# Yzmblog/SurfD

Measured on AMD Instinct MI355X. Metric: shapes/sec end-to-end (1000-step uncond, 512^3 UDF) at 1/2/4/8 GPU, higher is better.
Workload: dtype f32 (every matrix product of decoder and denoiser as three split-fp16 products on the fp16 MFMA pipe with fp32 accumulation — fp32-class error, same golden tolerances as the exact-fp32 kernels; samplers, attention, embedding MLP and grid bookkeeping in exact fp32)

## Files before the change

surfd_amd/csrc/unet.hip:

```cpp
#include "common.h"
#include "unet_api.h"
#include "unet_plan.h"
#include <string.h>
#include <algorithm>
#include <stdlib.h>

namespace surfd {

struct SegArgs {
    const float *x;
    long bstride;
    int C, Cp;
    int Lin;
    int taps, stride, ups;
    int gn, act;
    int bmod;
    const float *gamma, *beta;
    int kg_off;
    int cc;
    const float *add;
    long add_step_stride;
};

struct ConvArgs {
// ... 422 lines not shown
            const int ct = ct0 + i * ct_step;
            if (ct >= nct) continue;
            const int m = ct * 32 + (lane & 31);
            const bool mok = m < M;
            const int b = b0 + (m >> A.log2Lout), l = m & (A.Lout - 1);
            float add[16];
#pragma unroll
            for (int r = 0; r < 16; ++r) {
                if constexpr (NTW == 1) {
                    add[r] = pre_add[r];
                } else {
                    const int co = tile * 32 + frag_row(r, lane);
                    const bool ok = mok && co < A.Cout;
                    float t = 0.f;
                    if (ok) {
                        if (A.bias) t = A.bias[co];
                        if (embp) t += embp[b * A.emb_bstride + co];
                        if (A.res) t += A.res[b * A.res_bstride + (long)co * A.Lout + l];
                    }
                    add[r] = t;
                }
            }
#pragma unroll
            for (int r = 0; r < 16; ++r) {
                const int co = tile * 32 + frag_row(r, lane);
                if (mok && co < A.Cout) A.out[b * A.out_bstride + (long)co * A.Lout + l] = acc[i][r] + add[r];
            }
        }
    }
    if (dbg_on) { asm volatile("s_waitcnt vmcnt(0)" ::: "memory"); DBG_STAMP(9); }
#undef DBG_STAMP
}

__global__ __launch_bounds__(256) void attn_kernel(const float *qkv, long qkv_bstride, float *out, long out_bstride,
                                                   int heads, int d, int T, float scale) {
    extern __shared__ __attribute__((aligned(16))) float lds[];
    const int qt_n = (T + 31) >> 5;
    const int bh = blockIdx.x / qt_n, qt = blockIdx.x - bh * qt_n;
    const int b = bh / heads, h = bh - b * heads;
    const int tid = threadIdx.x, lane = tid & 63, col = lane & 31, half = lane >> 5;
    const int wave = __builtin_amdgcn_readfirstlane(tid >> 6);
    const int Tp = T + 1;
    float *q = lds, *k = q + d * Tp, *v = k + d * Tp;
    float *xch = v + d * Tp;
    if (T & 3) {
        const float *src = qkv + b * qkv_bstride + (long)h * 3 * d * T;
        for (int e = tid; e < 3 * d * T; e += 256) {
            const int c = e / T, t = e - c * T;
            lds[c * Tp + t] = c < 2 * d ? src[e] * scale : src[e];
        }
    } else {
        const f32x4 *src4 = reinterpret_cast<const f32x4 *>(qkv + b * qkv_bstride + (long)h * 3 * d * T);
        const int vpr = T >> 2, n4 = 3 * d * vpr;
        for (int e = tid; e < n4; e += 256) {
            const int c = e / vpr, t4 = e - c * vpr;
            f32x4 x = src4[e];
            if (c < 2 * d) { x[0] *= scale; x[1] *= scale; x[2] *= scale; x[3] *= scale; }
            float *dstp = lds + c * Tp + 4 * t4;
            dstp[0] = x[0]; dstp[1] = x[1]; dstp[2] = x[2]; dstp[3] = x[3];
        }
    }
    __syncthreads();
    const int t_glob = qt * 32 + col;
    const bool t_ok = t_glob < T;
    f32x16 sc[2];
#pragma unroll
    for (int kt = 0; kt < 2; ++kt)
#pragma unroll
        for (int r = 0; r < 16; ++r) sc[kt][r] = 0.f;
    const int cper = ((d / 2 + 3) / 4) * 2;
    const int c_beg = wave * cper, c_end = min(d, c_beg + cper);
    for (int c = c_beg; c < c_end; c += 2) {
        const float qv = t_ok ? q[(c + half) * Tp + t_glob] : 0.f;
#pragma unroll
        for (int kt = 0; kt < 2; ++kt)
            if (kt < qt_n) {
                const int s_ = kt * 32 + col;
                const float kv = s_ < T ? k[(c + half) * Tp + s_] : 0.f;
                sc[kt] = __builtin_amdgcn_mfma_f32_32x32x2f32(kv, qv, sc[kt], 0, 0, 0);
            }
    }
#pragma unroll
    for (int kt = 0; kt < 2; ++kt)
        if (kt < qt_n)
#pragma unroll
            for (int r = 0; r < 16; ++r) xch[((wave * qt_n + kt) * 16 + r) * 64 + lane] = sc[kt][r];
    __syncthreads();
#pragma unroll
    for (int kt = 0; kt < 2; ++kt)
        if (kt < qt_n)
#pragma unroll
            for (int r = 0; r < 16; ++r) {
                float t = 0.f;
#pragma unroll
                for (int w = 0; w < 4; ++w) t += xch[((w * qt_n + kt) * 16 + r) * 64 + lane];
                sc[kt][r] = t;
            }
    float mx = -INFINITY;
#pragma unroll
    for (int kt = 0; kt < 2; ++kt)
        if (kt < qt_n)
#pragma unroll
            for (int r = 0; r < 16; ++r) {
                const int s_ = kt * 32 + frag_row(r, lane);
                if (s_ >= T) sc[kt][r] = -INFINITY;
                mx = fmaxf(mx, sc[kt][r]);
            }
    mx = fmaxf(mx, __shfl_xor(mx, 32));
    float sum = 0.f;
#pragma unroll
    for (int kt = 0; kt < 2; ++kt)
        if (kt < qt_n)
#pragma unroll
            for (int r = 0; r < 16; ++r) { const float ex = expf(sc[kt][r] - mx); sc[kt][r] = ex; sum += ex; }
    sum += __shfl_xor(sum, 32);
#pragma unroll
    for (int kt = 0; kt < 2; ++kt)
#pragma unroll
        for (int r = 0; r < 16; ++r) sc[kt][r] = sc[kt][r] / sum;
    float *dst = out + b * out_bstride + (long)h * d * T;
    for (int c0 = wave * 32; c0 < d; c0 += 128) {
        f32x16 acc;
#pragma unroll
        for (int r = 0; r < 16; ++r) acc[r] = 0.f;
        const int c = c0 + col;
#pragma unroll
        for (int kt = 0; kt < 2; ++kt)
            if (kt < qt_n)
#pragma unroll
                for (int r = 0; r < 16; ++r) {
                    const int s_ = kt * 32 + frag_row(r, lane);
                    const float vv = (c < d && s_ < T) ? v[c * Tp + s_] : 0.f;
                    acc = __builtin_amdgcn_mfma_f32_32x32x2f32(vv, sc[kt][r], acc, 0, 0, 0);
                }
        if (t_ok)
#pragma unroll
            for (int r = 0; r < 16; ++r) {
                const int cr = c0 + frag_row(r, lane);
                if (cr < d) dst[(long)cr * T + t_glob] = acc[r];
            }
    }
}

__global__ void temb_kernel(const int64_t *t, int rows, int dim, float *out) {
    const int half = dim / 2;
    for (int e = blockIdx.x * blockDim.x + threadIdx.x; e < rows * half; e += gridDim.x * blockDim.x) {
        const int r = e / half, kk = e % half;
        const float freq = expf(__fdiv_rn(__fmul_rn(-9.210340371976184f, (float)kk), (float)half));
        const float a = __fmul_rn((float)t[r], freq);
        out[(long)r * dim + kk] = cosf(a);
        out[(long)r * dim + half + kk] = sinf(a);
    }
}

__global__ void add_label_kernel(float *emb, int rows, int dim, const float *table, const int64_t *cls, int B) {
    for (long e = blockIdx.x * (long)blockDim.x + threadIdx.x; e < (long)rows * dim; e += (long)gridDim.x * blockDim.x) {
        const int r = (int)(e / dim), c = (int)(e % dim);
        emb[e] += table[cls[r % B] * dim + c];
    }
}

__global__ void vec_add_kernel(float *dst, const float *a, const float *b, int n) {
    for (int e = blockIdx.x * blockDim.x + threadIdx.x; e < n; e += gridDim.x * blockDim.x) dst[e] = a[e] + (b ? b[e] : 0.f);
}

}

using namespace surfd;

namespace {

void add_param(surfd_unet *u, const std::string &k, std::vector<int64_t> shape) {
    u->pindex[k] = (int)u->params.size();
    u->params.push_back({k, std::move(shape)});
// ... 710 lines not shown
}

int unet_prepare_embeddings(surfd_unet *u, const int64_t *t_rows_host, int rows, const float *ctx, const int64_t *cls,
                            int B, hipStream_t st, bool shared) {
    if (rows > u->t_cap) {
        if (u->t_dev) HIP_TRY(hipFree(u->t_dev));
        u->t_dev = nullptr;
        HIP_TRY(hipMalloc((void **)&u->t_dev, (size_t)rows * sizeof(int64_t)));
        u->t_cap = rows;
    }
    HIP_TRY(hipMemcpyAsync(u->t_dev, t_rows_host, (size_t)rows * sizeof(int64_t), hipMemcpyHostToDevice, st));
    HIP_TRY(hipStreamSynchronize(st));
    return unet_prepare_embeddings_dev(u, u->t_dev, rows, ctx, cls, B, st, shared);
}

LoopState *unet_loop_state(surfd_unet *u) { return &u->loop; }
int unet_device(surfd_unet *u) { return u->device; }
long unet_workspace_generation(surfd_unet *u) { return u->ws_gen; }

static int run_op(surfd_unet *u, const Op &op, const float *x, float *out, int B, int L, const float *emb, hipStream_t st,
                  const int *step_ptr, const LoopFuse *lf = nullptr, bool *lf_done = nullptr) {
    if (op.kind == 0) {
        const float *in[2] = {x, x}; const long bs[2] = {(long)u->cfg.in_channels * L, (long)u->cfg.in_channels * L};
        const int bm[2] = {0, 0};
        return launch_conv(u, op.conv, B, L, in, bs, bm, out, (long)u->cfg.out_channels * L, emb, u->emb_total, st, step_ptr, lf, lf_done);
    }
    const AttnPlan &a = op.attn;
    const int T = L / a.ds, heads = u->cfg.num_heads, d = a.C / heads;
    const float *qkv = u->buf_ptr[a.qkv.buf];
    float *o = u->buf_ptr[a.out.buf];
    const long qbs = (long)u->bufs[a.qkv.buf].C * T, obs = (long)u->bufs[a.out.buf].C * T;
    const float scale = 1.f / sqrtf(sqrtf((float)d));
    if (T > 64) SURFD_FAIL(SURFD_ERR_UNSUPPORTED, "attention: sequence length %d (at most 64 positions per attention block)", T);
    const int qtn = (T + 31) / 32;
    const size_t lds_bytes = ((size_t)3 * d * (T + 1) + (size_t)4 * qtn * 16 * 64) * sizeof(float);
    hipLaunchKernelGGL(attn_kernel, dim3(B * heads * qtn), dim3(256), lds_bytes, st, qkv, qbs, o, obs, heads, d, T, scale);
    LAUNCH_CHECK();
    return SURFD_OK;
}

int unet_forward_prepared(surfd_unet *u, const float *x, int row0, float *out, int B, int L, hipStream_t st,
                          const int *step_ptr, const LoopFuse *lf, bool *lf_done) {
    if (!u->finalized) SURFD_FAIL(SURFD_ERR_STATE, "unet: parameters not finalized");
    if (row0 < 0 || row0 + (u->emb_shared ? 1 : B) > u->emb_rows) SURFD_FAIL(SURFD_ERR_STATE, "unet: embedding rows [%d,%d) not prepared", row0, row0 + B);
    if (u->emb_ingraph && (row0 != 0 || B != u->emb_B)) SURFD_FAIL(SURFD_ERR_STATE, "unet: in-loop embedding rows were prepared for %d samples", u->emb_B);
    int max_ds = 1;
    for (auto &b : u->bufs) max_ds = std::max(max_ds, b.ds);
    if (L % max_ds || L < max_ds || L > 64 || (L & (L - 1))) SURFD_FAIL(SURFD_ERR_UNSUPPORTED, "unet: latent length %d must be a power of two in [%d, 64]", L, max_ds);
    int rc = ensure_workspace(u, B, L);
    if (rc) return rc;
    const float *emb = u->emb_table + (size_t)row0 * u->emb_total;
    if (u->emb_ingraph) {
        const float *in[2] = {u->emb_ctx, nullptr}; const long bs[2] = {u->ted, 0}; const int bm[2] = {0, 0};
        if ((rc = launch_conv(u, u->lin3, B, 1, in, bs, bm, u->emb_table, u->emb_total, nullptr, 0, st, step_ptr, nullptr, nullptr, u->emb, u->ted))) return rc;
    }
    const ConvPlan *first_conv = nullptr;
    for (auto &op : u->ops) if (op.kind == 0) { first_conv = &op.conv; break; }
    for (size_t i = 0; i < u->ops.size(); ++i) {
        u->pf_next = first_conv;
        for (size_t j = i + 1; j < u->ops.size(); ++j) if (u->ops[j].kind == 0) { u->pf_next = &u->ops[j].conv; break; }
        rc = run_op(u, u->ops[i], x, out, B, L, emb, st, step_ptr, lf, lf_done);
        u->pf_next = nullptr;
        if (rc) return rc;
    }
    return SURFD_OK;
}
// ... 96 lines not shown
```

surfd_amd/csrc/decoder.hip:

```cpp
#include "common.h"
#include "points.h"
#include <string.h>
#include <stdlib.h>
#include <type_traits>
#include <utility>

namespace surfd {

constexpr int H = 512;
constexpr int NB = 5;
constexpr int NCBN = 2 * NB + 1;
constexpr int TP = 64;
constexpr int XS = H + 4;
constexpr int ES = 68;
constexpr int KG_H = H / 8;
constexpr int KG_E = 8;

constexpr size_t SZ_FCP = (size_t)16 * KG_E * 256;
constexpr size_t SZ_HH = (size_t)16 * KG_H * 256;
constexpr size_t SZ_FCPT = (size_t)2 * KG_H * 256;
constexpr size_t OFF_FCP = 0;
__host__ __device__ constexpr size_t off_fc(int k, int which) { return SZ_FCP + (size_t)(2 * k + which) * SZ_HH; }
__host__ __device__ constexpr size_t off_fcT(int k, int which) { return SZ_FCP + (size_t)(2 * NB + 2 * k + which) * SZ_HH; }
constexpr size_t OFF_FCPT = SZ_FCP + (size_t)4 * NB * SZ_HH;
constexpr size_t WPACK_FLOATS = OFF_FCPT + SZ_FCPT;
constexpr int VOFF_BFCP = 0;
__host__ __device__ constexpr int voff_bfc(int k, int which) { return H * (1 + 2 * k + which); }
constexpr int VOFF_WOUT = H * (1 + 2 * NB);
constexpr int VOFF_BOUT = H * (2 + 2 * NB);
__host__ __device__ constexpr int voff_cb(int k) { return VOFF_BOUT + 4 + H * k; }
constexpr int VEC_FLOATS = VOFF_BOUT + 4 + H * (NB + 1);

typedef _Float16 f16x8 __attribute__((ext_vector_type(8)));
typedef _Float16 f16x2 __attribute__((ext_vector_type(2)));
// ... 1002 lines not shown
    const __attribute__((address_space(1))) char *wb = (const __attribute__((address_space(1))) char *)(((unsigned long long)whi << 32) | wlo);
#pragma unroll
    for (int nt = 0; nt < 2; ++nt)
#pragma unroll
        for (int q = 0; q < 2; ++q)
#if defined(SURFD_DEC_W_NT) && SURFD_DEC_W_NT
            dst[nt][q] = __builtin_nontemporal_load(reinterpret_cast<const gf16x8 *>(wb + (size_t)(nt * KS * 2048) + (lofs + (unsigned)((ks * 2 + q) * 1024))));
#else
            dst[nt][q] = *reinterpret_cast<const gf16x8 *>(wb + (size_t)(nt * KS * 2048) + (lofs + (unsigned)((ks * 2 + q) * 1024)));
#endif
}

__device__ __forceinline__ void mfma_step8(const f16x8 (&a)[2][2], const f16x8 (&b)[2][2], f32x16 (&acc)[2][2]) {
    constexpr int TA[3] = {1, 0, 0};
    constexpr int TB[3] = {0, 1, 0};
#pragma unroll
    for (int t = 0; t < 3; ++t)
#pragma unroll
        for (int nt = 0; nt < 2; ++nt)
#pragma unroll
            for (int mt = 0; mt < 2; ++mt)
                acc[mt][nt] = __builtin_amdgcn_mfma_f32_32x32x16_f16(a[mt][TA[t]], b[nt][TB[t]], acc[mt][nt], 0, 0, 0);
}

template <int KS>
__device__ __forceinline__ void gemm8_request(WStages8 &ws, const _Float16 *Whf, int lane) {
    __builtin_amdgcn_sched_barrier(0);
    unsigned lofs = (unsigned)lane * 16u;
    asm volatile("" : "+v"(lofs));
    load_wstage8<KS>(ws.b[0], Whf, lofs, 0);
    __builtin_amdgcn_sched_barrier(0);
}

template <int KS>
__device__ __forceinline__ void gemm8(const float *A, const _Float16 *Whf, WStages8 &ws, f32x16 (&acc)[2][2], int lane) {
    constexpr int D = 4;
    static_assert(KS % D == 0, "k-step count must be a multiple of the pipeline depth");
    const float *a0 = A + (lane & 31) * XS + 4 * (lane >> 5);
    const float *a1 = a0 + 32 * XS;
    unsigned lofs = (unsigned)lane * 16u;
    asm volatile("" : "+v"(lofs));
    f16x8 x[2][2][2];
    auto group = [&](int ks0, auto last) {
        int goff = ks0 * 8;
        asm volatile("" : "+v"(goff));
#pragma unroll
        for (int j = 0; j < D; ++j) {
            if (!decltype(last)::value || j == 0) load_wstage8<KS>(ws.b[(j + D - 1) % D], Whf, lofs, ks0 + j + D - 1);
            const int jn = (decltype(last)::value && j == D - 1) ? j : j + 1;
            x[(j + 1) & 1][0][0] = *reinterpret_cast<const f16x8 *>(a0 + goff + jn * 8); x[(j + 1) & 1][0][1] = *reinterpret_cast<const f16x8 *>(a0 + goff + 256 + jn * 8);
            x[(j + 1) & 1][1][0] = *reinterpret_cast<const f16x8 *>(a1 + goff + jn * 8); x[(j + 1) & 1][1][1] = *reinterpret_cast<const f16x8 *>(a1 + goff + 256 + jn * 8);
            mfma_step8(x[j & 1], ws.b[j], acc);
#pragma unroll
            for (int i = 0; i < 4; ++i) { __builtin_amdgcn_sched_group_barrier(0x008, 1, 0); __builtin_amdgcn_sched_group_barrier(0x020, 1, 0); }
#pragma unroll
            for (int i = 0; i < 4; ++i) { __builtin_amdgcn_sched_group_barrier(0x008, 1, 0); __builtin_amdgcn_sched_group_barrier(0x100, 1, 0); }
            __builtin_amdgcn_sched_group_barrier(0x008, 4, 0);
            __builtin_amdgcn_sched_barrier(0);
        }
    };
    x[0][0][0] = *reinterpret_cast<const f16x8 *>(a0); x[0][0][1] = *reinterpret_cast<const f16x8 *>(a0 + 256);
    x[0][1][0] = *reinterpret_cast<const f16x8 *>(a1); x[0][1][1] = *reinterpret_cast<const f16x8 *>(a1 + 256);
    if constexpr (KS > D) {
#pragma unroll
        for (int d = 1; d < D - 1; ++d) load_wstage8<KS>(ws.b[d], Whf, lofs, d);
#pragma unroll 1
        for (int ks0 = 0; ks0 < KS - D; ks0 += D) group(ks0, std::false_type{});
        group(KS - D, std::true_type{});
    } else {
#pragma unroll
        for (int d = 1; d < D; ++d) load_wstage8<KS>(ws.b[d], Whf, lofs, d);
        int goff = 0;
        asm volatile("" : "+v"(goff));
#pragma unroll
        for (int j = 0; j < D; ++j) {
            const int jn = j == D - 1 ? j : j + 1;
            x[(j + 1) & 1][0][0] = *reinterpret_cast<const f16x8 *>(a0 + goff + jn * 8); x[(j + 1) & 1][0][1] = *reinterpret_cast<const f16x8 *>(a0 + goff + 256 + jn * 8);
            x[(j + 1) & 1][1][0] = *reinterpret_cast<const f16x8 *>(a1 + goff + jn * 8); x[(j + 1) & 1][1][1] = *reinterpret_cast<const f16x8 *>(a1 + goff + 256 + jn * 8);
            mfma_step8(x[j & 1], ws.b[j], acc);
            __builtin_amdgcn_sched_barrier(0);
        }
    }
}

__global__ __launch_bounds__(512, 1) void decoder_fwd8_kernel(DecParams P, PtBatch B) {
    extern __shared__ __attribute__((aligned(16))) float lds[];
    float *X = lds;
    float *PT = lds + TP * XS;
    float *LOG = PT + TP * 4;
    const int tid = threadIdx.x, lane = tid & 63, wave = tid >> 6;
    const int col = lane & 31;
    const int wave_u = __builtin_amdgcn_readfirstlane(wave);
    float *const xb0 = X + (4 * (lane >> 5)) * XS + 64 * wave + col;
    float *const xb1 = xb0 + 32 * XS;
#define XAT8(mt, nt, r) ((mt) ? xb1 : xb0)[(((r) & 3) + 8 * ((r) >> 2)) * XS + 32 * (nt)]
    typedef unsigned __attribute__((address_space(3))) lds_u32;
    lds_u32 *xw0 = (lds_u32 *)(reinterpret_cast<unsigned *>(X) + (4 * (lane >> 5)) * XS + 32 * wave + col);
    lds_u32 *xw1 = xw0 + 32 * XS;
#define XW8(mt, r, pl) ((mt) ? xw1 : xw0)[(((r) & 3) + 8 * ((r) >> 2)) * XS + 256 * (pl)]
#ifndef SURFD_DEC_XCD_STAGGER
#define SURFD_DEC_XCD_STAGGER 0
#endif
#if SURFD_DEC_XCD_STAGGER > 0
    for (int k_ = 0; k_ < (int)(blockIdx.x & 7) * SURFD_DEC_XCD_STAGGER; ++k_) __builtin_amdgcn_s_sleep(127);
#endif
#ifndef SURFD_DEC_CLOCK
#define SURFD_DEC_CLOCK 1
#endif
#if SURFD_DEC_CLOCK
    unsigned long long *const clk = reinterpret_cast<unsigned long long *>(P.sat + 2);
    unsigned long long *const clk0 = reinterpret_cast<unsigned long long *>(LOG + TP);
    if (blockIdx.x == 0 && tid == 0) {
        clk0[0] = (unsigned long long)__builtin_readcyclecounter();
        clk0[1] = (unsigned long long)__builtin_amdgcn_s_memrealtime();
    }
#endif
    int sat_flag = 0;
    auto store8 = [&](const f32x16 (&v)[2][2], const float (&sa)[2], const float (&sb)[2]) {
        float umax = 0.f;
#pragma unroll
        for (int mt = 0; mt < 2; ++mt)
#pragma unroll
            for (int r = 0; r < 16; ++r) {
                const float t0 = __builtin_fmaf(sa[0], v[mt][0][r], sb[0]);
                const float t1 = __builtin_fmaf(sa[1], v[mt][1][r], sb[1]);
                umax = __builtin_fmaxf(__builtin_fmaxf(umax, t0), t1);
                const float u0 = __builtin_amdgcn_fmed3f(t0, 0.f, 65504.f);
                const float u1 = __builtin_amdgcn_fmed3f(t1, 0.f, 65504.f);
                const f32x2 u = {u0, u1};
                const unsigned h = __builtin_bit_cast(unsigned, __builtin_convertvector(u, f16x2));
                XW8(mt, r, 0) = h;
                XW8(mt, r, 1) = split_low_pair(h, u0, u1);
            }
        sat_flag |= __any(umax > 65504.f);
    };
    auto zero8 = [](f32x16 (&a)[2][2]) {
#pragma unroll
        for (int mt = 0; mt < 2; ++mt)
#pragma unroll
            for (int nt = 0; nt < 2; ++nt)
#pragma unroll
                for (int r = 0; r < 16; ++r) a[mt][nt][r] = 0.f;
    };
    WStages8 ws;
    for (int bi = 0; bi < B.n; ++bi) {
    const PtIO &io = B.io[bi];
    const long npts = pt_count(io);
    const long ntiles = (npts + TP - 1) / TP;
    const float *tab_sample = P.tab + (size_t)B.sample[bi] * NCBN * 2 * H;
    const long tstep = io.shard_n > 1 ? io.shard_n : 1;
    for (long tile = blockIdx.x * tstep + (io.shard_n > 1 ? io.shard_i : 0); tile < ntiles; tile += gridDim.x * tstep) {
        const long e0 = tile * TP;
        const float *vecs_ = P.vecs, *tab_ = tab_sample;
        const _Float16 *whf = P.whf;
        unsigned cb = 64 * wave + col;
        asm volatile("" : "+s"(vecs_), "+s"(tab_), "+s"(whf), "+v"(cb), "+v"(xw0), "+v"(xw1));
        const gfloat *vecs = (const gfloat *)vecs_, *tab = (const gfloat *)tab_;
        const size_t woff_e = (size_t)(2 * wave_u) * KS_E * 2 * 512, woff = (size_t)(2 * wave_u) * KS_H * 2 * 512;
        __syncthreads();
        {
        int tid_fe = threadIdx.x;
        asm volatile("" : "+v"(tid_fe));
        const int tid = tid_fe;
        if (tid < TP) {
            const long e = e0 + tid;
            float x = 0.f, y = 0.f, z = 0.f;
            int vox = -1;
            if (e < npts) {
                if (io.mode == PT_XYZ) { x = io.xyz[e * 3 + 0]; y = io.xyz[e * 3 + 1]; z = io.xyz[e * 3 + 2]; vox = 0; }
                else if (io.mode == PT_EMB) vox = 0;
                else { vox = pt_voxel(io, e); voxel_xyz(io, vox, x, y, z); }
            }
            PT[tid * 4 + 0] = x; PT[tid * 4 + 1] = y; PT[tid * 4 + 2] = z;
            PT[tid * 4 + 3] = __int_as_float(vox);
        }
        __syncthreads();
        encode_tile_f16x2<8>(io, e0, npts, PT, X, tid, sat_flag);
        }
        gemm8_request<KS_E>(ws, whf + woff_e, lane);
        __syncthreads();
        f32x16 net[2][2], tmp[2][2];
        zero8(net);
        const float winv = vecs[VOFF_SC + 1];
        float nsa[2], nsb[2];
#pragma unroll
        for (int nt = 0; nt < 2; ++nt) {
            const unsigned c = cb + 32 * nt;
            const float a = tab[c];
            nsa[nt] = a * winv;
            nsb[nt] = __builtin_fmaf(a, vecs[voff_cb(0) + c], tab[H + c]);
        }
        gemm8<KS_E>(X, whf + woff_e, ws, net, lane);
        __syncthreads();
#pragma unroll 1
        for (int k = 0; k < NB; ++k) {
            const _Float16 *W0 = whf + (HF_FCP + (size_t)(2 * k) * HF_HH) + woff, *W1 = W0 + HF_HH;
            {
                float sa[2] = {nsa[0], nsa[1]}, sb[2] = {nsb[0], nsb[1]};
                store8(net, sa, sb);
            }
            gemm8_request<KS_H>(ws, W0, lane);
            __syncthreads();
            zero8(tmp);
            float sa1[2], sbb[2];
#pragma unroll
            for (int nt = 0; nt < 2; ++nt) {
                const unsigned c = cb + 32 * nt;
                const float a = tab[(2 * k + 1) * 2 * H + c];
                sa1[nt] = a * winv;
                sbb[nt] = __builtin_fmaf(a, vecs[H * (1 + 2 * k) + c], tab[(2 * k + 1) * 2 * H + H + c]);
            }
            gemm8<KS_H>(X, W0, ws, tmp, lane);
            __syncthreads();
            store8(tmp, sa1, sbb);
            gemm8_request<KS_H>(ws, W1, lane);
            __syncthreads();
#pragma unroll
            for (int nt = 0; nt < 2; ++nt) {
                const unsigned c = cb + 32 * nt;
                const float a = tab[(2 * k + 2) * 2 * H + c];
                nsa[nt] = a * winv;
                nsb[nt] = __builtin_fmaf(a, vecs[voff_cb(0) + H * (k + 1) + c], tab[(2 * k + 2) * 2 * H + H + c]);
            }
            gemm8<KS_H>(X, W1, ws, net, lane);
            __syncthreads();
        }
        {
#pragma unroll
            for (int nt = 0; nt < 2; ++nt) {
                const float wo = vecs[VOFF_WOUT + cb + 32 * nt];
#pragma unroll
                for (int mt = 0; mt < 2; ++mt)
#pragma unroll
                    for (int r = 0; r < 16; ++r) {
                        const float u = nsa[nt] * net[mt][nt][r] + nsb[nt];
                        XAT8(mt, nt, r) = fmaxf(u, 0.f) * wo;
                    }
            }
        }
        __syncthreads();
        {
            const float bo = vecs[VOFF_BOUT];
            for (int pp = 0; pp < TP / 8; ++pp) {
                const int p = wave * (TP / 8) + pp;
                float sacc = 0.f;
#pragma unroll
                for (int i = 0; i < H / 64; ++i) sacc += X[p * XS + lane + 64 * i];
#pragma unroll
                for (int off = 32; off > 0; off >>= 1) sacc += __shfl_xor(sacc, off);
                if (lane == 0) LOG[p] = sacc + bo;
            }
        }
        __syncthreads();
        if (tid < TP) {
            const long e = e0 + tid;
            const bool valid = e < npts;
            float udf = 0.f;
            int vox = 0;
            if (valid) {
                const float o = LOG[tid];
                const float y = 1.f / (1.f + expf(-o));
                udf = (1.f - y) * 0.1f;
                if (io.out_logit) io.out_logit[e] = o;
                if (io.out_udf) io.out_udf[e] = udf;
                if (io.grid_udf) {
                    vox = __float_as_int(PT[tid * 4 + 3]);
                    io.grid_udf[vox] = udf;
                }
            }
            if (io.grid_udf && io.grad_list) {
                const int slot = wave_append_slot(io.grad_count, valid && udf < io.grad_thr);
                if (slot >= 0) io.grad_list[slot] = vox;
            }
        }
    }
    }
    if (sat_flag && lane == 0) atomicAdd(P.sat, 1u);
#if SURFD_DEC_CLOCK
    if (blockIdx.x == 0 && tid == 0) {
        const unsigned long long c1 = (unsigned long long)__builtin_readcyclecounter(), r1 = (unsigned long long)__builtin_amdgcn_s_memrealtime();
        atomicAdd(clk + 2, c1 - clk0[0]);
        atomicAdd(clk + 3, r1 - clk0[1]);
    }
#endif
}
#undef XAT8
#undef XW8

#undef XW
constexpr size_t DEC_LDS_BYTES = (size_t)(TP * XS + TP * 4 + TP + TP * ES + TP * 4 + 4) * sizeof(float);

__global__ void absmax_kernel(const float *src, size_t n, unsigned *out) {
    unsigned m = 0u;
    for (size_t i = blockIdx.x * (size_t)blockDim.x + threadIdx.x; i < n; i += (size_t)gridDim.x * blockDim.x)
        m = max(m, __float_as_uint(src[i]) & 0x7fffffffu);
#pragma unroll
    for (int off = 32; off > 0; off >>= 1) m = max(m, (unsigned)__shfl_xor((int)m, off));
    if ((threadIdx.x & 63) == 0 && m) atomicMax(out, m);
}

__global__ void weight_scale_kernel(const unsigned *maxbits, float *sc) {
    const unsigned b = *maxbits;
    int e = (int)(b >> 23) - 127;
    if (b == 0u || e > 100 || e < -100) e = 8;
    sc[0] = __uint_as_float((unsigned)(127 + 8 - e) << 23);
    sc[1] = __uint_as_float((unsigned)(127 - 8 + e) << 23);
}
// ... 454 lines not shown
```

Before: 4.924.

## Specialize attention kernel on sequence length and batch LDS loads

Moves the attention body into a templated core specialized by sequence length, so that only the needed score fragment rows are reduced, exponentiated and multiplied for short sequences. The global-to-LDS staging now issues four loads per thread before any stores and uses shift and mask indexing in place of division. The QK loop preloads eight channel pairs from LDS ahead of the MFMAs, and waves that own no output channels exit after the exchange barrier. A power-of-two check on T is added to protect the shift indexing. Attention is a small share of the UNet, so the end-to-end effect is likely limited.

```diff
diff --git a/surfd_amd/csrc/unet.hip b/surfd_amd/csrc/unet.hip
--- a/surfd_amd/csrc/unet.hip
+++ b/surfd_amd/csrc/unet.hip
@@ -478,114 +478,155 @@
 #undef DBG_STAMP
 }
 
+template <int NR, int KT, class Sink>
+__device__ __forceinline__ void attn_core_tile(float *lds, const float *src, int d, int T, int qt, float scale, Sink &&sink) {
+    constexpr int qt_n = KT;
+    const int tid = threadIdx.x, lane = tid & 63, col = lane & 31, half = lane >> 5;
+    const int wave = __builtin_amdgcn_readfirstlane(tid >> 6);
+    const int Tp = T + 1;
+    float *q = lds, *k = q + d * Tp, *v = k + d * Tp;
+    float *xch = v + d * Tp;
+    if (T & 3) {
+        const int lt = __builtin_ctz(T), n = 3 * d * T;
+        for (int e0 = tid; e0 < n; e0 += 1024) {
+            float x[4];
+#pragma unroll
+            for (int j = 0; j < 4; ++j) x[j] = src[min(e0 + 256 * j, n - 1)];
+#pragma unroll
+            for (int j = 0; j < 4; ++j) asm volatile("" : "+v"(x[j]));
+#pragma unroll
+            for (int j = 0; j < 4; ++j) {
+                const int e = e0 + 256 * j;
+                const int c = e >> lt, t = e & (T - 1);
+                if (e < n) lds[c * Tp + t] = c < 2 * d ? x[j] * scale : x[j];
+            }
+        }
+    } else {
+        const f32x4 *src4 = reinterpret_cast<const f32x4 *>(src);
+        const int vpr = T >> 2, lv = __builtin_ctz(vpr), n4 = 3 * d * vpr;
+        for (int e0 = tid; e0 < n4; e0 += 1024) {
+            f32x4 xs[4];
+#pragma unroll
+            for (int j = 0; j < 4; ++j) xs[j] = src4[min(e0 + 256 * j, n4 - 1)];
+#pragma unroll
+            for (int j = 0; j < 4; ++j) asm volatile("" : "+v"(xs[j]));
+#pragma unroll
+            for (int j = 0; j < 4; ++j) {
+                const int e = e0 + 256 * j;
+                const int c = e >> lv, t4 = e & (vpr - 1);
+                f32x4 x = xs[j];
+                if (c < 2 * d) { x[0] *= scale; x[1] *= scale; x[2] *= scale; x[3] *= scale; }
+                if (e < n4) {
+                    float *dstp = lds + c * Tp + 4 * t4;
+                    dstp[0] = x[0]; dstp[1] = x[1]; dstp[2] = x[2]; dstp[3] = x[3];
+                }
+            }
+        }
+    }
+    __syncthreads();
+    const int t_glob = qt * 32 + col;
+    const bool t_ok = t_glob < T;
+    f32x16 sc[KT];
+#pragma unroll
+    for (int kt = 0; kt < KT; ++kt)
+#pragma unroll
+        for (int r = 0; r < 16; ++r) sc[kt][r] = 0.f;
+    const int cper = ((d / 2 + 3) / 4) * 2;
+    const int c_beg = wave * cper, c_end = min(d, c_beg + cper);
+    const int c_last = c_beg + ((c_end - 1 - c_beg) & ~1);
+    for (int c0 = c_beg; c0 < c_end; c0 += 16) {
+        float qv[8], kv[8][KT];
+#pragma unroll
+        for (int i = 0; i < 8; ++i) {
+            const int c = min(c0 + 2 * i, c_last);
+            qv[i] = t_ok ? q[(c + half) * Tp + t_glob] : 0.f;
+#pragma unroll
+            for (int kt = 0; kt < KT; ++kt) {
+                const int s_ = kt * 32 + col;
+                kv[i][kt] = s_ < T ? k[(c + half) * Tp + s_] : 0.f;
+            }
+        }
+#pragma unroll
+        for (int i = 0; i < 8; ++i)
+            if (c0 + 2 * i < c_end) {
+#pragma unroll
+                for (int kt = 0; kt < KT; ++kt) sc[kt] = __builtin_amdgcn_mfma_f32_32x32x2f32(kv[i][kt], qv[i], sc[kt], 0, 0, 0);
+            }
+    }
+#pragma unroll
+    for (int kt = 0; kt < KT; ++kt)
+#pragma unroll
+        for (int r = 0; r < (kt ? 16 : NR); ++r) xch[((wave * qt_n + kt) * 16 + r) * 64 + lane] = sc[kt][r];
+    __syncthreads();
+    if (wave * 32 >= d) return;
+#pragma unroll
+    for (int kt = 0; kt < KT; ++kt)
+#pragma unroll
+        for (int r = 0; r < (kt ? 16 : NR); ++r) {
+            float t = 0.f;
+#pragma unroll
+            for (int w = 0; w < 4; ++w) t += xch[((w * qt_n + kt) * 16 + r) * 64 + lane];
+            sc[kt][r] = t;
+        }
+    float mx = -INFINITY;
+#pragma unroll
+    for (int kt = 0; kt < KT; ++kt)
+#pragma unroll
+        for (int r = 0; r < (kt ? 16 : NR); ++r) {
+            const int s_ = kt * 32 + frag_row(r, lane);
+            if (s_ >= T) sc[kt][r] = -INFINITY;
+            mx = fmaxf(mx, sc[kt][r]);
+        }
+    mx = fmaxf(mx, __shfl_xor(mx, 32));
+    float sum = 0.f;
+#pragma unroll
+    for (int kt = 0; kt < KT; ++kt)
+#pragma unroll
+        for (int r = 0; r < (kt ? 16 : NR); ++r) { const float ex = expf(sc[kt][r] - mx); sc[kt][r] = ex; sum += ex; }
+    sum += __shfl_xor(sum, 32);
+#pragma unroll
+    for (int kt = 0; kt < KT; ++kt)
+#pragma unroll
+        for (int r = 0; r < (kt ? 16 : NR); ++r) sc[kt][r] = sc[kt][r] / sum;
+    for (int c0 = wave * 32; c0 < d; c0 += 128) {
+        f32x16 acc;
+#pragma unroll
+        for (int r = 0; r < 16; ++r) acc[r] = 0.f;
+        const int c = c0 + col;
+#pragma unroll
+        for (int kt = 0; kt < KT; ++kt)
+#pragma unroll
+            for (int r = 0; r < (kt ? 16 : NR); ++r) {
+                const int s_ = kt * 32 + frag_row(r, lane);
+                const float vv = (c < d && s_ < T) ? v[c * Tp + s_] : 0.f;
+                acc = __builtin_amdgcn_mfma_f32_32x32x2f32(vv, sc[kt][r], acc, 0, 0, 0);
+            }
+        if (t_ok)
+#pragma unroll
+            for (int r = 0; r < 16; ++r) {
+                const int cr = c0 + frag_row(r, lane);
+                if (cr < d) sink(cr, t_glob, acc[r]);
+            }
+    }
+}
+
+template <class Sink>
+__device__ __forceinline__ void attn_core(float *lds, const float *src, int d, int T, int qt, float scale, Sink &&sink) {
+    if (T > 32) attn_core_tile<16, 2>(lds, src, d, T, qt, scale, sink);
+    else if (T > 16) attn_core_tile<16, 1>(lds, src, d, T, qt, scale, sink);
+    else if (T > 8) attn_core_tile<8, 1>(lds, src, d, T, qt, scale, sink);
+    else attn_core_tile<4, 1>(lds, src, d, T, qt, scale, sink);
+}
+
 __global__ __launch_bounds__(256) void attn_kernel(const float *qkv, long qkv_bstride, float *out, long out_bstride,
                                                    int heads, int d, int T, float scale) {
     extern __shared__ __attribute__((aligned(16))) float lds[];
     const int qt_n = (T + 31) >> 5;
     const int bh = blockIdx.x / qt_n, qt = blockIdx.x - bh * qt_n;
     const int b = bh / heads, h = bh - b * heads;
-    const int tid = threadIdx.x, lane = tid & 63, col = lane & 31, half = lane >> 5;
-    const int wave = __builtin_amdgcn_readfirstlane(tid >> 6);
-    const int Tp = T + 1;
-    float *q = lds, *k = q + d * Tp, *v = k + d * Tp;
-    float *xch = v + d * Tp;
-    if (T & 3) {
-        const float *src = qkv + b * qkv_bstride + (long)h * 3 * d * T;
-        for (int e = tid; e < 3 * d * T; e += 256) {
-            const int c = e / T, t = e - c * T;
-            lds[c * Tp + t] = c < 2 * d ? src[e] * scale : src[e];
-        }
-    } else {
-        const f32x4 *src4 = reinterpret_cast<const f32x4 *>(qkv + b * qkv_bstride + (long)h * 3 * d * T);
-        const int vpr = T >> 2, n4 = 3 * d * vpr;
-        for (int e = tid; e < n4; e += 256) {
-            const int c = e / vpr, t4 = e - c * vpr;
-            f32x4 x = src4[e];
-            if (c < 2 * d) { x[0] *= scale; x[1] *= scale; x[2] *= scale; x[3] *= scale; }
-            float *dstp = lds + c * Tp + 4 * t4;
-            dstp[0] = x[0]; dstp[1] = x[1]; dstp[2] = x[2]; dstp[3] = x[3];
-        }
-    }
-    __syncthreads();
-    const int t_glob = qt * 32 + col;
-    const bool t_ok = t_glob < T;
-    f32x16 sc[2];
-#pragma unroll
-    for (int kt = 0; kt < 2; ++kt)
-#pragma unroll
-        for (int r = 0; r < 16; ++r) sc[kt][r] = 0.f;
-    const int cper = ((d / 2 + 3) / 4) * 2;
-    const int c_beg = wave * cper, c_end = min(d, c_beg + cper);
-    for (int c = c_beg; c < c_end; c += 2) {
-        const float qv = t_ok ? q[(c + half) * Tp + t_glob] : 0.f;
-#pragma unroll
-        for (int kt = 0; kt < 2; ++kt)
-            if (kt < qt_n) {
-                const int s_ = kt * 32 + col;
-                const float kv = s_ < T ? k[(c + half) * Tp + s_] : 0.f;
-                sc[kt] = __builtin_amdgcn_mfma_f32_32x32x2f32(kv, qv, sc[kt], 0, 0, 0);
-            }
-    }
-#pragma unroll
-    for (int kt = 0; kt < 2; ++kt)
-        if (kt < qt_n)
-#pragma unroll
-            for (int r = 0; r < 16; ++r) xch[((wave * qt_n + kt) * 16 + r) * 64 + lane] = sc[kt][r];
-    __syncthreads();
-#pragma unroll
-    for (int kt = 0; kt < 2; ++kt)
-        if (kt < qt_n)
-#pragma unroll
-            for (int r = 0; r < 16; ++r) {
-                float t = 0.f;
-#pragma unroll
-                for (int w = 0; w < 4; ++w) t += xch[((w * qt_n + kt) * 16 + r) * 64 + lane];
-                sc[kt][r] = t;
-            }
-    float mx = -INFINITY;
-#pragma unroll
-    for (int kt = 0; kt < 2; ++kt)
-        if (kt < qt_n)
-#pragma unroll
-            for (int r = 0; r < 16; ++r) {
-                const int s_ = kt * 32 + frag_row(r, lane);
-                if (s_ >= T) sc[kt][r] = -INFINITY;
-                mx = fmaxf(mx, sc[kt][r]);
-            }
-    mx = fmaxf(mx, __shfl_xor(mx, 32));
-    float sum = 0.f;
-#pragma unroll
-    for (int kt = 0; kt < 2; ++kt)
-        if (kt < qt_n)
-#pragma unroll
-            for (int r = 0; r < 16; ++r) { const float ex = expf(sc[kt][r] - mx); sc[kt][r] = ex; sum += ex; }
-    sum += __shfl_xor(sum, 32);
-#pragma unroll
-    for (int kt = 0; kt < 2; ++kt)
-#pragma unroll
-        for (int r = 0; r < 16; ++r) sc[kt][r] = sc[kt][r] / sum;
     float *dst = out + b * out_bstride + (long)h * d * T;
-    for (int c0 = wave * 32; c0 < d; c0 += 128) {
-        f32x16 acc;
-#pragma unroll
-        for (int r = 0; r < 16; ++r) acc[r] = 0.f;
-        const int c = c0 + col;
-#pragma unroll
-        for (int kt = 0; kt < 2; ++kt)
-            if (kt < qt_n)
-#pragma unroll
-                for (int r = 0; r < 16; ++r) {
-                    const int s_ = kt * 32 + frag_row(r, lane);
-                    const float vv = (c < d && s_ < T) ? v[c * Tp + s_] : 0.f;
-                    acc = __builtin_amdgcn_mfma_f32_32x32x2f32(vv, sc[kt][r], acc, 0, 0, 0);
-                }
-        if (t_ok)
-#pragma unroll
-            for (int r = 0; r < 16; ++r) {
-                const int cr = c0 + frag_row(r, lane);
-                if (cr < d) dst[(long)cr * T + t_glob] = acc[r];
-            }
-    }
+    attn_core(lds, qkv + b * qkv_bstride + (long)h * 3 * d * T, d, T, qt, scale,
+              [&](int c, int t, float a) { dst[(long)c * T + t] = a; });
 }
 
 __global__ void temb_kernel(const int64_t *t, int rows, int dim, float *out) {
@@ -1362,6 +1403,7 @@
     const long qbs = (long)u->bufs[a.qkv.buf].C * T, obs = (long)u->bufs[a.out.buf].C * T;
     const float scale = 1.f / sqrtf(sqrtf((float)d));
     if (T > 64) SURFD_FAIL(SURFD_ERR_UNSUPPORTED, "attention: sequence length %d (at most 64 positions per attention block)", T);
+    if (T < 1 || (T & (T - 1))) SURFD_FAIL(SURFD_ERR_UNSUPPORTED, "attention: sequence length %d is not a power of two", T);
     const int qtn = (T + 31) / 32;
     const size_t lds_bytes = ((size_t)3 * d * (T + 1) + (size_t)4 * qtn * 16 * 64) * sizeof(float);
     hipLaunchKernelGGL(attn_kernel, dim3(B * heads * qtn), dim3(256), lds_bytes, st, qkv, qbs, o, obs, heads, d, T, scale);
```

After: 4.948 (median of 6 runs). About the same (+0.5%).

## Skew decoder wave groups by one interval to overlap epilogue stores with MFMA

Applied to the files above, without the earlier changes.

The decoder's per-tile layer loop is replaced by a compile-time schedule from a new header. The header splits the eight waves into two groups, one lagging the other by one barrier interval, and splits each hidden GEMM into two K halves. The aim is for one group's LDS epilogue writes and weight requests to run while the other group is on the MFMA pipe, so the block no longer sits idle at every barrier. In exchange it adds idle slots for the lag, more barriers per tile, and a constexpr-checked region-ownership scheme whose correctness depends on the half-split access pattern.

```diff
diff --git a/surfd_amd/csrc/decoder.hip b/surfd_amd/csrc/decoder.hip
--- a/surfd_amd/csrc/decoder.hip
+++ b/surfd_amd/csrc/decoder.hip
@@ -1,5 +1,6 @@
 #include "common.h"
 #include "points.h"
+#include "decoder_sched.h"
 #include <string.h>
 #include <stdlib.h>
 #include <type_traits>
@@ -1068,22 +1069,22 @@
     __builtin_amdgcn_sched_barrier(0);
 }
 
-template <int KS>
-__device__ __forceinline__ void gemm8(const float *A, const _Float16 *Whf, WStages8 &ws, f32x16 (&acc)[2][2], int lane) {
-    constexpr int D = 4;
-    static_assert(KS % D == 0, "k-step count must be a multiple of the pipeline depth");
+template <int KS, int BEG>
+__device__ __forceinline__ void gemm8_half(const float *A, const _Float16 *Whf, WStages8 &ws, f32x16 (&acc)[2][2], int lane) {
+    constexpr int D = 4, END = BEG + KS / 2;
+    static_assert((KS / 2) % D == 0 && KS / 2 > D && (BEG == 0 || BEG == KS / 2), "two halves of whole pipeline groups");
     const float *a0 = A + (lane & 31) * XS + 4 * (lane >> 5);
     const float *a1 = a0 + 32 * XS;
     unsigned lofs = (unsigned)lane * 16u;
     asm volatile("" : "+v"(lofs));
     f16x8 x[2][2][2];
-    auto group = [&](int ks0, auto last) {
+    auto group = [&](int ks0, auto last_x, auto last_w) {
         int goff = ks0 * 8;
         asm volatile("" : "+v"(goff));
 #pragma unroll
         for (int j = 0; j < D; ++j) {
-            if (!decltype(last)::value || j == 0) load_wstage8<KS>(ws.b[(j + D - 1) % D], Whf, lofs, ks0 + j + D - 1);
-            const int jn = (decltype(last)::value && j == D - 1) ? j : j + 1;
+            if (!decltype(last_w)::value || j == 0) load_wstage8<KS>(ws.b[(j + D - 1) % D], Whf, lofs, ks0 + j + D - 1);
+            const int jn = (decltype(last_x)::value && j == D - 1) ? j : j + 1;
             x[(j + 1) & 1][0][0] = *reinterpret_cast<const f16x8 *>(a0 + goff + jn * 8); x[(j + 1) & 1][0][1] = *reinterpret_cast<const f16x8 *>(a0 + goff + 256 + jn * 8);
             x[(j + 1) & 1][1][0] = *reinterpret_cast<const f16x8 *>(a1 + goff + jn * 8); x[(j + 1) & 1][1][1] = *reinterpret_cast<const f16x8 *>(a1 + goff + 256 + jn * 8);
             mfma_step8(x[j & 1], ws.b[j], acc);
@@ -1095,27 +1096,38 @@
             __builtin_amdgcn_sched_barrier(0);
         }
     };
+    x[0][0][0] = *reinterpret_cast<const f16x8 *>(a0 + BEG * 8); x[0][0][1] = *reinterpret_cast<const f16x8 *>(a0 + BEG * 8 + 256);
+    x[0][1][0] = *reinterpret_cast<const f16x8 *>(a1 + BEG * 8); x[0][1][1] = *reinterpret_cast<const f16x8 *>(a1 + BEG * 8 + 256);
+    if constexpr (BEG == 0) {
+#pragma unroll
+        for (int d = 1; d < D - 1; ++d) load_wstage8<KS>(ws.b[d], Whf, lofs, d);
+    }
+#pragma unroll 1
+    for (int ks0 = BEG; ks0 < END - D; ks0 += D) group(ks0, std::false_type{}, std::false_type{});
+    group(END - D, std::true_type{}, std::integral_constant<bool, END == KS>{});
+}
+
+__device__ __forceinline__ void gemm8_e(const float *A, const _Float16 *Whf, WStages8 &ws, f32x16 (&acc)[2][2], int lane) {
+    constexpr int D = 4, KS = KS_E;
+    static_assert(KS == D, "one pipeline group");
+    const float *a0 = A + (lane & 31) * XS + 4 * (lane >> 5);
+    const float *a1 = a0 + 32 * XS;
+    unsigned lofs = (unsigned)lane * 16u;
+    asm volatile("" : "+v"(lofs));
+    f16x8 x[2][2][2];
     x[0][0][0] = *reinterpret_cast<const f16x8 *>(a0); x[0][0][1] = *reinterpret_cast<const f16x8 *>(a0 + 256);
     x[0][1][0] = *reinterpret_cast<const f16x8 *>(a1); x[0][1][1] = *reinterpret_cast<const f16x8 *>(a1 + 256);
-    if constexpr (KS > D) {
-#pragma unroll
-        for (int d = 1; d < D - 1; ++d) load_wstage8<KS>(ws.b[d], Whf, lofs, d);
-#pragma unroll 1
-        for (int ks0 = 0; ks0 < KS - D; ks0 += D) group(ks0, std::false_type{});
-        group(KS - D, std::true_type{});
-    } else {
-#pragma unroll
-        for (int d = 1; d < D; ++d) load_wstage8<KS>(ws.b[d], Whf, lofs, d);
-        int goff = 0;
-        asm volatile("" : "+v"(goff));
-#pragma unroll
-        for (int j = 0; j < D; ++j) {
-            const int jn = j == D - 1 ? j : j + 1;
-            x[(j + 1) & 1][0][0] = *reinterpret_cast<const f16x8 *>(a0 + goff + jn * 8); x[(j + 1) & 1][0][1] = *reinterpret_cast<const f16x8 *>(a0 + goff + 256 + jn * 8);
-            x[(j + 1) & 1][1][0] = *reinterpret_cast<const f16x8 *>(a1 + goff + jn * 8); x[(j + 1) & 1][1][1] = *reinterpret_cast<const f16x8 *>(a1 + goff + 256 + jn * 8);
-            mfma_step8(x[j & 1], ws.b[j], acc);
-            __builtin_amdgcn_sched_barrier(0);
-        }
+#pragma unroll
+    for (int d = 1; d < D; ++d) load_wstage8<KS>(ws.b[d], Whf, lofs, d);
+    int goff = 0;
+    asm volatile("" : "+v"(goff));
+#pragma unroll
+    for (int j = 0; j < D; ++j) {
+        const int jn = j == D - 1 ? j : j + 1;
+        x[(j + 1) & 1][0][0] = *reinterpret_cast<const f16x8 *>(a0 + goff + jn * 8); x[(j + 1) & 1][0][1] = *reinterpret_cast<const f16x8 *>(a0 + goff + 256 + jn * 8);
+        x[(j + 1) & 1][1][0] = *reinterpret_cast<const f16x8 *>(a1 + goff + jn * 8); x[(j + 1) & 1][1][1] = *reinterpret_cast<const f16x8 *>(a1 + goff + 256 + jn * 8);
+        mfma_step8(x[j & 1], ws.b[j], acc);
+        __builtin_amdgcn_sched_barrier(0);
     }
 }
 
@@ -1127,8 +1139,6 @@
     const int tid = threadIdx.x, lane = tid & 63, wave = tid >> 6;
     const int col = lane & 31;
     const int wave_u = __builtin_amdgcn_readfirstlane(wave);
-    float *const xb0 = X + (4 * (lane >> 5)) * XS + 64 * wave + col;
-    float *const xb1 = xb0 + 32 * XS;
 #define XAT8(mt, nt, r) ((mt) ? xb1 : xb0)[(((r) & 3) + 8 * ((r) >> 2)) * XS + 32 * (nt)]
     typedef unsigned __attribute__((address_space(3))) lds_u32;
     lds_u32 *xw0 = (lds_u32 *)(reinterpret_cast<unsigned *>(X) + (4 * (lane >> 5)) * XS + 32 * wave + col);
@@ -1193,122 +1203,153 @@
         asm volatile("" : "+s"(vecs_), "+s"(tab_), "+s"(whf), "+v"(cb), "+v"(xw0), "+v"(xw1));
         const gfloat *vecs = (const gfloat *)vecs_, *tab = (const gfloat *)tab_;
         const size_t woff_e = (size_t)(2 * wave_u) * KS_E * 2 * 512, woff = (size_t)(2 * wave_u) * KS_H * 2 * 512;
-        __syncthreads();
-        {
-        int tid_fe = threadIdx.x;
-        asm volatile("" : "+v"(tid_fe));
-        const int tid = tid_fe;
-        if (tid < TP) {
-            const long e = e0 + tid;
-            float x = 0.f, y = 0.f, z = 0.f;
-            int vox = -1;
-            if (e < npts) {
-                if (io.mode == PT_XYZ) { x = io.xyz[e * 3 + 0]; y = io.xyz[e * 3 + 1]; z = io.xyz[e * 3 + 2]; vox = 0; }
-                else if (io.mode == PT_EMB) vox = 0;
-                else { vox = pt_voxel(io, e); voxel_xyz(io, vox, x, y, z); }
-            }
-            PT[tid * 4 + 0] = x; PT[tid * 4 + 1] = y; PT[tid * 4 + 2] = z;
-            PT[tid * 4 + 3] = __int_as_float(vox);
-        }
-        __syncthreads();
-        encode_tile_f16x2<8>(io, e0, npts, PT, X, tid, sat_flag);
-        }
-        gemm8_request<KS_E>(ws, whf + woff_e, lane);
-        __syncthreads();
-        f32x16 net[2][2], tmp[2][2];
-        zero8(net);
         const float winv = vecs[VOFF_SC + 1];
-        float nsa[2], nsb[2];
-#pragma unroll
-        for (int nt = 0; nt < 2; ++nt) {
-            const unsigned c = cb + 32 * nt;
-            const float a = tab[c];
-            nsa[nt] = a * winv;
-            nsb[nt] = __builtin_fmaf(a, vecs[voff_cb(0) + c], tab[H + c]);
-        }
-        gemm8<KS_E>(X, whf + woff_e, ws, net, lane);
-        __syncthreads();
+        auto run_tile = [&](auto group_c) {
+            namespace S = fwd8;
+            constexpr int G = decltype(group_c)::value;
+            static_assert(S::equal_barrier_counts() && S::rows_are_loops(G) && S::layers_are_contiguous(G) && S::NLAYER == 2 * NB,
+                          "decoder_sched.h: a row must be prologue, NB times the same six phases, epilogue, with as many intervals as the other row");
+            constexpr int LB = S::loop_begin(G), LE = S::loop_end(G), N = S::SCHED.n[G];
+            f32x16 net[2][2], tmp[2][2];
+            float nsa[2], nsb[2], sa1[2], sbb[2];
+            auto phase = [&](auto phase_c, auto second_c, int k) {
+                constexpr int PH = decltype(phase_c)::value;
+                constexpr bool SECOND = decltype(second_c)::value;
+                if constexpr (PH == S::FETCH) {
+                    int tid_f = threadIdx.x;
+                    asm volatile("" : "+v"(tid_f));
+                    const int tid = tid_f;
+                    if (tid < TP) {
+                        const long e = e0 + tid;
+                        float x = 0.f, y = 0.f, z = 0.f;
+                        int vox = -1;
+                        if (e < npts) {
+                            if (io.mode == PT_XYZ) { x = io.xyz[e * 3 + 0]; y = io.xyz[e * 3 + 1]; z = io.xyz[e * 3 + 2]; vox = 0; }
+                            else if (io.mode == PT_EMB) vox = 0;
+                            else { vox = pt_voxel(io, e); voxel_xyz(io, vox, x, y, z); }
+                        }
+                        PT[tid * 4 + 0] = x; PT[tid * 4 + 1] = y; PT[tid * 4 + 2] = z;
+                        PT[tid * 4 + 3] = __int_as_float(vox);
+                    }
+                } else if constexpr (PH == S::ENCODE) {
+                    int tid_e = threadIdx.x;
+                    asm volatile("" : "+v"(tid_e));
+                    encode_tile_f16x2<8>(io, e0, npts, PT, X, tid_e, sat_flag);
+                    gemm8_request<KS_E>(ws, whf + woff_e, lane);
+                } else if constexpr (PH == S::GEMM_E) {
+                    zero8(net);
+#pragma unroll
+                    for (int nt = 0; nt < 2; ++nt) {
+                        const unsigned c = cb + 32 * nt;
+                        const float a = tab[c];
+                        nsa[nt] = a * winv;
+                        nsb[nt] = __builtin_fmaf(a, vecs[voff_cb(0) + c], tab[H + c]);
+                    }
+                    gemm8_e(X, whf + woff_e, ws, net, lane);
+                } else if constexpr (PH == S::EPI) {
+                    if constexpr (!SECOND) store8(net, nsa, nsb);
+                    else store8(tmp, sa1, sbb);
+                    gemm8_request<KS_H>(ws, whf + (HF_FCP + (size_t)(2 * k + (SECOND ? 1 : 0)) * HF_HH) + woff, lane);
+                } else if constexpr (PH == S::GEMM_H1 || PH == S::GEMM_H2) {
+                    const _Float16 *W = whf + (HF_FCP + (size_t)(2 * k + (SECOND ? 1 : 0)) * HF_HH) + woff;
+                    if constexpr (PH == S::GEMM_H1) {
+                        if constexpr (!SECOND) zero8(tmp);
+#pragma unroll
+                        for (int nt = 0; nt < 2; ++nt) {
+                            const unsigned c = cb + 32 * nt;
+                            if constexpr (!SECOND) {
+                                const float a = tab[(2 * k + 1) * 2 * H + c];
+                                sa1[nt] = a * winv;
+                                sbb[nt] = __builtin_fmaf(a, vecs[H * (1 + 2 * k) + c], tab[(2 * k + 1) * 2 * H + H + c]);
+                            } else {
+                                const float a = tab[(2 * k + 2) * 2 * H + c];
+                                nsa[nt] = a * winv;
+                                nsb[nt] = __builtin_fmaf(a, vecs[voff_cb(0) + H * (k + 1) + c], tab[(2 * k + 2) * 2 * H + H + c]);
+                            }
+                        }
+                    }
+                    constexpr int BEG = PH == S::GEMM_H1 ? 0 : KS_H / 2;
+                    if constexpr (!SECOND) gemm8_half<KS_H, BEG>(X, W, ws, tmp, lane);
+                    else gemm8_half<KS_H, BEG>(X, W, ws, net, lane);
+                } else if constexpr (PH == S::FINAL) {
+                    int tid_x = threadIdx.x;
+                    asm volatile("" : "+v"(tid_x));
+                    float *const xb0 = X + (4 * ((tid_x & 63) >> 5)) * XS + 64 * (tid_x >> 6) + (tid_x & 31);
+                    float *const xb1 = xb0 + 32 * XS;
+#pragma unroll
+                    for (int nt = 0; nt < 2; ++nt) {
+                        const float wo = vecs[VOFF_WOUT + cb + 32 * nt];
+#pragma unroll
+                        for (int mt = 0; mt < 2; ++mt)
+#pragma unroll
+                            for (int r = 0; r < 16; ++r) {
+                                const float u = nsa[nt] * net[mt][nt][r] + nsb[nt];
+                                XAT8(mt, nt, r) = fmaxf(u, 0.f) * wo;
+                            }
+                    }
+                } else if constexpr (PH == S::REDUCE) {
+                    const float bo = vecs[VOFF_BOUT];
+                    int tid_r = threadIdx.x;
+                    asm volatile("" : "+v"(tid_r));
+                    const int lane = tid_r & 63, wave = tid_r >> 6;
+                    for (int pp = 0; pp < TP / 8; ++pp) {
+                        const int p = wave * (TP / 8) + pp;
+                        float sacc = 0.f;
+#pragma unroll
+                        for (int i = 0; i < H / 64; ++i) sacc += X[p * XS + lane + 64 * i];
+#pragma unroll
+                        for (int off = 32; off > 0; off >>= 1) sacc += __shfl_xor(sacc, off);
+                        if (lane == 0) LOG[p] = sacc + bo;
+                    }
+                } else if constexpr (PH == S::OUTPUT) {
+                    int tid_o = threadIdx.x;
+                    asm volatile("" : "+v"(tid_o));
+                    const int tid = tid_o;
+                    if (tid < TP) {
+                        const long e = e0 + tid;
+                        const bool valid = e < npts;
+                        float udf = 0.f;
+                        int vox = 0;
+                        if (valid) {
+                            const float o = LOG[tid];
+                            const float y = 1.f / (1.f + expf(-o));
+                            udf = (1.f - y) * 0.1f;
+                            if (io.out_logit) io.out_logit[e] = o;
+                            if (io.out_udf) io.out_udf[e] = udf;
+                            if (io.grid_udf) {
+                                vox = __float_as_int(PT[tid * 4 + 3]);
+                                io.grid_udf[vox] = udf;
+                            }
+                        }
+                        if (io.grid_udf && io.grad_list) {
+                            const int slot = wave_append_slot(io.grad_count, valid && udf < io.grad_thr);
+                            if (slot >= 0) io.grad_list[slot] = vox;
+                        }
+                    }
+                } else {
+                    static_assert(PH == S::IDLE, "a phase without code");
+                }
+            };
+            static_for<LB>([&](auto t) {
+                constexpr S::Slot s = S::SCHED.s[G][decltype(t)::value];
+                __syncthreads();
+                phase(std::integral_constant<int, s.phase>{}, std::false_type{}, 0);
+            });
 #pragma unroll 1
-        for (int k = 0; k < NB; ++k) {
-            const _Float16 *W0 = whf + (HF_FCP + (size_t)(2 * k) * HF_HH) + woff, *W1 = W0 + HF_HH;
-            {
-                float sa[2] = {nsa[0], nsa[1]}, sb[2] = {nsb[0], nsb[1]};
-                store8(net, sa, sb);
-            }
-            gemm8_request<KS_H>(ws, W0, lane);
-            __syncthreads();
-            zero8(tmp);
-            float sa1[2], sbb[2];
-#pragma unroll
-            for (int nt = 0; nt < 2; ++nt) {
-                const unsigned c = cb + 32 * nt;
-                const float a = tab[(2 * k + 1) * 2 * H + c];
-                sa1[nt] = a * winv;
-                sbb[nt] = __builtin_fmaf(a, vecs[H * (1 + 2 * k) + c], tab[(2 * k + 1) * 2 * H + H + c]);
-            }
-            gemm8<KS_H>(X, W0, ws, tmp, lane);
-            __syncthreads();
-            store8(tmp, sa1, sbb);
-            gemm8_request<KS_H>(ws, W1, lane);
-            __syncthreads();
-#pragma unroll
-            for (int nt = 0; nt < 2; ++nt) {
-                const unsigned c = cb + 32 * nt;
-                const float a = tab[(2 * k + 2) * 2 * H + c];
-                nsa[nt] = a * winv;
-                nsb[nt] = __builtin_fmaf(a, vecs[voff_cb(0) + H * (k + 1) + c], tab[(2 * k + 2) * 2 * H + H + c]);
-            }
-            gemm8<KS_H>(X, W1, ws, net, lane);
-            __syncthreads();
-        }
-        {
-#pragma unroll
-            for (int nt = 0; nt < 2; ++nt) {
-                const float wo = vecs[VOFF_WOUT + cb + 32 * nt];
-#pragma unroll
-                for (int mt = 0; mt < 2; ++mt)
-#pragma unroll
-                    for (int r = 0; r < 16; ++r) {
-                        const float u = nsa[nt] * net[mt][nt][r] + nsb[nt];
-                        XAT8(mt, nt, r) = fmaxf(u, 0.f) * wo;
-                    }
-            }
-        }
-        __syncthreads();
-        {
-            const float bo = vecs[VOFF_BOUT];
-            for (int pp = 0; pp < TP / 8; ++pp) {
-                const int p = wave * (TP / 8) + pp;
-                float sacc = 0.f;
-#pragma unroll
-                for (int i = 0; i < H / 64; ++i) sacc += X[p * XS + lane + 64 * i];
-#pragma unroll
-                for (int off = 32; off > 0; off >>= 1) sacc += __shfl_xor(sacc, off);
-                if (lane == 0) LOG[p] = sacc + bo;
-            }
-        }
-        __syncthreads();
-        if (tid < TP) {
-            const long e = e0 + tid;
-            const bool valid = e < npts;
-            float udf = 0.f;
-            int vox = 0;
-            if (valid) {
-                const float o = LOG[tid];
-                const float y = 1.f / (1.f + expf(-o));
-                udf = (1.f - y) * 0.1f;
-                if (io.out_logit) io.out_logit[e] = o;
-                if (io.out_udf) io.out_udf[e] = udf;
-                if (io.grid_udf) {
-                    vox = __float_as_int(PT[tid * 4 + 3]);
-                    io.grid_udf[vox] = udf;
-                }
-            }
-            if (io.grid_udf && io.grad_list) {
-                const int slot = wave_append_slot(io.grad_count, valid && udf < io.grad_thr);
-                if (slot >= 0) io.grad_list[slot] = vox;
-            }
-        }
+            for (int k = 0; k < NB; ++k)
+                static_for<S::BLOCK_INTERVALS>([&](auto i) {
+                    constexpr S::Slot s = S::SCHED.s[G][LB + decltype(i)::value];
+                    __syncthreads();
+                    phase(std::integral_constant<int, s.phase>{}, std::integral_constant<bool, s.layer == 2>{}, k);
+                });
+            static_for<N - LE>([&](auto t) {
+                constexpr S::Slot s = S::SCHED.s[G][LE + decltype(t)::value];
+                __syncthreads();
+                phase(std::integral_constant<int, s.phase>{}, std::false_type{}, 0);
+            });
+        };
+        if (wave_u < 4) run_tile(std::integral_constant<int, 0>{});
+        else run_tile(std::integral_constant<int, 1>{});
     }
     }
     if (sat_flag && lane == 0) atomicAdd(P.sat, 1u);
diff --git a/surfd_amd/csrc/decoder_sched.h b/surfd_amd/csrc/decoder_sched.h
--- /dev/null
+++ b/surfd_amd/csrc/decoder_sched.h
@@ -0,0 +1,125 @@
+#pragma once
+
+namespace surfd {
+namespace fwd8 {
+
+enum Phase : int {
+    IDLE = 0,
+    FETCH,
+    ENCODE,
+    GEMM_E,
+    EPI,
+    GEMM_H1,
+    GEMM_H2,
+    FINAL,
+    REDUCE,
+    OUTPUT
+};
+
+struct Slot { int phase, layer; };
+
+constexpr int NGROUP = 2;
+constexpr int NLAYER = 10;
+constexpr int LAG[NGROUP] = {0, 1};
+constexpr int MAXLAG = 1;
+constexpr int MAXINT = 48;
+
+struct Sched { Slot s[NGROUP][MAXINT]; int n[NGROUP]; };
+
+constexpr Sched make_sched() {
+    Sched r{};
+    for (int g = 0; g < NGROUP; ++g) {
+        int t = 0;
+        r.s[g][t++] = Slot{g == 0 ? FETCH : IDLE, 0};
+        r.s[g][t++] = Slot{ENCODE, 0};
+        r.s[g][t++] = Slot{GEMM_E, 0};
+        for (int i = 0; i < LAG[g]; ++i) r.s[g][t++] = Slot{IDLE, 0};
+        for (int l = 1; l <= NLAYER; ++l) {
+            r.s[g][t++] = Slot{EPI, l};
+            r.s[g][t++] = Slot{GEMM_H1, l};
+            r.s[g][t++] = Slot{GEMM_H2, l};
+        }
+        for (int i = LAG[g]; i < MAXLAG; ++i) r.s[g][t++] = Slot{IDLE, 0};
+        r.s[g][t++] = Slot{FINAL, 0};
+        r.s[g][t++] = Slot{REDUCE, 0};
+        r.s[g][t++] = Slot{g == 0 ? OUTPUT : IDLE, 0};
+        r.n[g] = t;
+    }
+    return r;
+}
+constexpr Sched SCHED = make_sched();
+
+constexpr int BLOCK_INTERVALS = 6;
+constexpr int loop_begin(int g) {
+    int t = 0;
+    while (t < SCHED.n[g] && SCHED.s[g][t].phase != EPI) ++t;
+    return t;
+}
+constexpr int loop_end(int g) { return loop_begin(g) + BLOCK_INTERVALS * (NLAYER / 2); }
+constexpr bool hidden(int phase) { return phase == EPI || phase == GEMM_H1 || phase == GEMM_H2; }
+constexpr bool rows_are_loops(int g) {
+    const int lb = loop_begin(g), le = loop_end(g);
+    if (le > SCHED.n[g]) return false;
+    for (int t = 0; t < SCHED.n[g]; ++t) {
+        const Slot s = SCHED.s[g][t];
+        if (t < lb || t >= le) {
+            if (hidden(s.phase)) return false;
+            continue;
+        }
+        const int k = (t - lb) / BLOCK_INTERVALS, i = (t - lb) % BLOCK_INTERVALS;
+        const Slot first = SCHED.s[g][lb + i];
+        if (s.phase != first.phase || s.layer != first.layer + 2 * k || !hidden(s.phase)) return false;
+        if (first.layer != 1 + i / 3) return false;
+    }
+    return true;
+}
+constexpr bool layers_are_contiguous(int g) {
+    for (int t = 0; t < SCHED.n[g]; ++t) {
+        const Slot s = SCHED.s[g][t];
+        if (s.phase == EPI && !(t + 1 < SCHED.n[g] && SCHED.s[g][t + 1].phase == GEMM_H1 && SCHED.s[g][t + 1].layer == s.layer)) return false;
+        if (s.phase == GEMM_H1 && !(t + 1 < SCHED.n[g] && SCHED.s[g][t + 1].phase == GEMM_H2 && SCHED.s[g][t + 1].layer == s.layer)) return false;
+        if (s.phase == GEMM_E && !(t > 0 && SCHED.s[g][t - 1].phase == ENCODE)) return false;
+    }
+    return true;
+}
+constexpr bool equal_barrier_counts() {
+    for (int g = 1; g < NGROUP; ++g)
+        if (SCHED.n[g] != SCHED.n[0]) return false;
+    return true;
+}
+
+enum Region : unsigned {
+    X_H1_HI = 1u << 0, X_H2_HI = 1u << 1, X_H1_LO = 1u << 2, X_H2_LO = 1u << 3, R_PT = 1u << 4, R_LOG = 1u << 5
+};
+constexpr int NREGION = 6;
+constexpr unsigned X_H1 = X_H1_HI | X_H1_LO, X_H2 = X_H2_HI | X_H2_LO, X_ALL = X_H1 | X_H2;
+
+struct Access { unsigned reads, writes; };
+constexpr Access access(int g, int phase) {
+    switch (phase) {
+        case FETCH: return Access{0u, R_PT};
+        case ENCODE: return Access{R_PT, X_H1};
+        case GEMM_E: return Access{X_H1, 0u};
+        case EPI: return Access{0u, g == 0 ? X_H1 : X_H2};
+        case GEMM_H1: return Access{X_H1, 0u};
+        case GEMM_H2: return Access{X_H2, 0u};
+        case FINAL: return Access{0u, g == 0 ? (X_H1_HI | X_H2_HI) : (X_H1_LO | X_H2_LO)};
+        case REDUCE: return Access{X_ALL, R_LOG};
+        case OUTPUT: return Access{R_LOG | R_PT, 0u};
+        default: return Access{0u, 0u};
+    }
+}
+constexpr bool cooperative(int phase) { return phase == ENCODE || phase == REDUCE; }
+constexpr Slot needs(int phase, int layer, unsigned r) {
+    switch (phase) {
+        case ENCODE: return Slot{FETCH, 0};
+        case GEMM_E: return Slot{ENCODE, 0};
+        case GEMM_H1: case GEMM_H2: return Slot{EPI, layer};
+        case REDUCE: return Slot{FINAL, 0};
+        case OUTPUT: return (r == R_LOG) ? Slot{REDUCE, 0} : Slot{FETCH, 0};
+        default: return Slot{IDLE, 0};
+    }
+}
+
+}
+}
```

Measured after the change: 4.896 before, 4.910 after, median of 6. Within noise of the previous version (+0.3%).
